# hku-mars/LiDAR_IMU_Init

Hardware: AMD Instinct MI355X
Metric: ICP+ESKF scans/sec @100k pts/scan (higher is better)
Workload: dtype f64; 1 GPU; stream100k: 100000 pts/scan (time-sorted) vs 1000000-pt local map, max_iteration 5, LIO mode (12-col H), static map, voxel-grid leaf 0.05; scans resident in HBM, 8 distinct scans cycled, the state reset to the scan's propagated state every step; map_points=1000000, params=harness/launch/ouster (reference-format yaml + launch), parallelism=points sharded x1, transport=none, rccl_ranks=0

## Files before the change

lidar_imu_init_amd/csrc/lii_capi.cpp:

```cpp
#include "lii_context.h"

using namespace lii_impl;

namespace lii_impl {

thread_local std::string g_err;

static constexpr unsigned kProfEventFlags = hipEventDisableSystemFence;

void harvest_knn_events(lii_handle h) {
  const unsigned int due = h->prof.ev_it_due;
  h->prof.ev_it_due = 0u;
  for (int it = 0; it < 16; it++) {
    if (!((due >> it) & 1u)) continue;
    float kk = 0;
    if (hipEventElapsedTime(&kk, h->prof.ev_it[2 * it], h->prof.ev_it[2 * it + 1]) != hipSuccess) continue;
    h->prof.timings[7] += kk;
    h->prof.timings[5] += 1;
  }
}

int fail(lii_handle h, int code, const std::string& msg) {
  if (h) h->err = msg;
  g_err = msg;
// ... 49 lines not shown
  return rb;
}
PoseArg pose_of(const lii_state& s) {
  PoseArg p;
  std::memcpy(p.R, s.rot_end, 72);
  std::memcpy(p.p, s.pos_end, 24);
  std::memcpy(p.RLI, s.offset_R_L_I, 72);
  std::memcpy(p.TLI, s.offset_T_L_I, 24);
  return p;
}
bool fuse_filter(lii_handle h, float leaf) {
  if (!(leaf > 0.f) || h->voxel_sort || h->no_fuse) return false;
  if (h->vh.part_world > 1) return true;
  return h->vh_mode == 1 && (h->vh_pinned || leaf == h->vh_leaf);
}
DeskewPlan deskew_plan(lii_handle h, const float4* in, float4* out, int n, bool sorted, const unsigned long long* extent, float leaf, bool fused,
                       DeskewCtrl ctrl) {
  DeskewPlan dp = {};
  dp.in = in; dp.out = out; dp.n = n; dp.sorted = sorted ? 1 : 0; dp.extent = extent; dp.bbox_rows = h->d_bbox_rows;
  dp.leaf = leaf; dp.vh = fused ? &h->vh : nullptr;
  if (ctrl == DeskewCtrl::pulled) { dp.ctrl_src = h->h_ctrl; dp.ctrl_dst = h->d_ctrl; dp.ctrl_bytes = (sizeof(IekfCtrl) + 15) / 16 * 16; }
#ifdef LII_GAP_TRACE
  if (ctrl != DeskewCtrl::none) dp.gap = h->d_gran;
#endif
  return dp;
}
int resolve_n_body(lii_handle h) {
  if (!h->n_body_pending) return LII_OK;
  int* v = h->h_small->n_body;
  HIPCHK(h, hipMemcpyAsync(v, h->d_nbody, 2 * sizeof(int), hipMemcpyDeviceToHost, h->stream));
  HIPCHK(h, hipStreamSynchronize(h->stream));
  h->n_body = v[0];
// ... 767 lines not shown
  unsigned int* mm = h->d_mm + 8 * h->mm_sel;
  if (h->bbox_rows == 0) {
    h->mm_sel ^= 1;
    launch_voxel_minmax(h->d_scan, n, mm, h->d_mm + 8 * h->mm_sel, s);
  }
  h->vh_calls++;
  if (h->vh_flag_pending && h->vh_calls >= h->vh_due) {
    HIPCHK(h, hipEventSynchronize(h->ev_vh));
    h->vh_flag_pending = false;
    if (h->vh_mode == 0 && *h->h_vh_crowded <= 32u) h->vh_mode = 1;
    else if (h->vh_mode == 1 && *h->h_vh_crowded > 64u) h->vh_mode = 0;
  }
  int hash_stages = 3;
  const bool inserted = h->vh_inserted;
  h->vh_inserted = false;
  if (inserted && leaf != h->vh_inserted_leaf) return fail(h, LII_ERR_STATE, "lii_downsample: the de-skew prepared the voxel filter for another leaf size");
  if (inserted) hash_stages = 4;
  if (!inserted && !h->vh_pinned && !h->voxel_sort && leaf != h->vh_leaf) {
    h->vh_leaf = leaf;
    h->vh_flag_pending = false;
    HIPCHK(h, hipMemsetAsync(h->vh.crowded, 0, sizeof(unsigned int), s));
    launch_voxel_hash(h->vh, h->d_scan, n, mm, h->d_bbox_rows, h->bbox_rows, leaf, h->d_body, h->d_nbody, h->d_nbody + 1, h->d_vpcl_out, 1, 0u, s);
    HIPCHK(h, hipMemcpyAsync(h->h_vh_crowded, h->vh.crowded, sizeof(unsigned int), hipMemcpyDeviceToHost, s));
    HIPCHK(h, hipMemsetAsync(h->vh.crowded, 0, sizeof(unsigned int), s));
    HIPCHK(h, hipStreamSynchronize(s));
    h->vh_mode = *h->h_vh_crowded > 32u ? 0 : 1;
    hash_stages = 2;
    if (h->vh_mode == 0)
      launch_voxel_hash_clear(h->vh, voxel_hash_slots(n), s);
  }
  const bool use_hash = inserted || (h->vh_mode == 1 && !h->voxel_sort);
  h->voxel_path_hash = use_hash;
  const bool by_voxel = inserted && h->vh.part_world > 1;
  if (use_hash) {
    if (++h->vh_epoch == 0u) h->vh_epoch = 1u;
    launch_voxel_hash(h->vh, h->d_scan, n, mm, h->d_bbox_rows, h->bbox_rows, leaf, h->d_body, h->d_nbody, h->d_nbody + 1, h->d_vpcl_out, hash_stages, h->vh_epoch, s, h->test_emit_late ? 1 : 0, inten, inten_out);
    if (!h->vh_pinned && !by_voxel && !h->vh_flag_pending && (++h->vh_watch & 15) == 0) {
      HIPCHK(h, hipMemcpyAsync(h->h_vh_crowded, h->vh.crowded, sizeof(unsigned int), hipMemcpyDeviceToHost, s));
      HIPCHK(h, hipMemsetAsync(h->vh.crowded, 0, sizeof(unsigned int), s));
      HIPCHK(h, hipEventRecord(h->ev_vh, s));
      h->vh_flag_pending = true;
      h->vh_due = h->vh_calls + 8;
    }
  } else {
    const VoxelSortPlan plan = voxel_sort_plan(n);
    launch_voxel_keys(h->d_scan, n, mm, h->d_bbox_rows, h->bbox_rows, leaf, h->d_vkeys_a, h->d_vpcl_in,
                      h->d_nbody + 1, plan.samples ? h->d_vsplit + 2048 : nullptr, plan.width, s);
    VoxelSortBuffers vb;
    vb.pcl_in = h->d_vpcl_in; vb.pcl_out = h->d_vpcl_out;
    vb.samples = h->d_vsplit + 2048;
    vb.keys_in = h->d_vkeys_a; vb.keys_out = h->d_vkeys_b; vb.idx_out = h->d_vidx_b;
// ... 150 lines not shown
```

lidar_imu_init_amd/csrc/lii_capi_register.cpp:

```cpp
#include "lii_context.h"
#include <cstddef>

#include "lii_hostmath.h"

using namespace lii_impl;

namespace {

int next_knn_epoch(lii_handle h) {
  h->knn_epoch = h->knn_epoch >= 0x3FFFFFFE ? 1 : h->knn_epoch + 1;
  return h->knn_epoch;
}
void launch_knn(lii_handle h, const GridView& g, const RegistrationBuffers& rb, const PoseArg* pose, int forced, int epoch,
                hipEvent_t ev_start = nullptr, hipEvent_t ev_stop = nullptr) {
  lii::launch_knn(g, rb, pose, h->d_ctrl, forced, h->d_ctrl->search_pose, h->stream, epoch, ev_start, ev_stop);
}

void note_noise_pass(lii_handle h) { if (h->noise.model == 1) h->noise.have_pass = true; }

int iterate(lii_handle h, const lii_state* st, bool search, bool imu_en, double* out91) {
  if (h->n_body <= 0) return fail(h, LII_ERR_STATE, "no down-sampled scan (call lii_downsample / lii_downsample_skip)");
  int rc = commit_map(h);
  if (rc != LII_OK) return rc;
  if (!search && !h->have_search) return fail(h, LII_ERR_STATE, "non-search iteration before any search");
// ... 102 lines not shown
void run_wait_hook(lii_handle h, bool inside) {
  if (!h->wait_hook) return;
  void (*hook)(void*) = h->wait_hook;
  h->wait_hook = nullptr;
  if (inside) h->in_wait_hook = true;
  hook(h->wait_hook_arg);
  if (inside) h->in_wait_hook = false;
}

struct DevicePasses {
  lii_handle h; const lii_iekf_opts* opts; hipStream_t s;
  GridView g; RegistrationBuffers rb;
  const PoseArg* pose;
  bool prof;
  unsigned int plan;

  int enqueue(int it) {
    const bool knn = it >= 16 || ((plan >> it) & 1u);
    const int epoch = knn ? next_knn_epoch(h) : 0;
    if (knn) {
      if (h->prof.kp_active) { const int r = kp_mark(h, LII_KP_KNN, it); if (r != LII_OK) return r; }
      if (prof && it < 16) launch_knn(h, g, rb, pose, -1, epoch, h->prof.ev_it[2 * it], h->prof.ev_it[2 * it + 1]);
      else launch_knn(h, g, rb, pose, -1, epoch);
    }
    if (h->prof.kp_active) { const int r = kp_mark(h, LII_KP_FIT, it); if (r != LII_OK) return r; }
    if (knn && h->wide_listed && !h->net.comm && h->net.n_ranks <= 1) launch_complete_listed(g, rb, h->d_ctrl, -1, s, epoch);
    launch_fit_reduce(g, rb, pose, h->d_ctrl, -1, opts->imu_en ? 1 : 0, h->cfg.plane_threshold, h->cfg.laser_point_cov_inv, s, epoch);
    note_noise_pass(h);
    if (h->prof.kp_active) { const int r = kp_mark(h, LII_KP_SOLVE, it); if (r != LII_OK) return r; }
    if (!h->net.comm) {
      launch_reduce_solve(rb, h->d_gran, h->d_ctrl, h->h_res, mailbox_view(h), s, epoch);
      return LII_OK;
    }
    launch_reduce91(rb, h->d_out91, h->d_ctrl, -1, s, epoch);
    ncclResult_t r = ncclAllReduce(h->d_out91, h->d_out91 + 128, kNormalEq, ncclDouble, ncclSum, h->net.comm, s);
    if (r != ncclSuccess) return fail(h, LII_ERR_COMM, std::string("ncclAllReduce: ") + ncclGetErrorString(r));
    launch_iekf_solve(h->d_ctrl, h->d_out91 + 128, h->h_res, s);
    return LII_OK;
  }

  int wait() {
    const int parked_word = h->update_seq | kLoopParked;
    if (h->poll_result && !h->net.comm) {
      volatile int* done = &h->h_res->done;
      unsigned int spins = 0;
// ... 136 lines not shown
  if (!h->ctrl_preloaded) {
    if (h->staging_busy) HIPCHK(h, hipStreamSynchronize(s));
    fill_ctrl(h, state, state_prop, opts);
    HIPCHK(h, hipMemcpyAsync(h->d_ctrl, h->h_ctrl, sizeof(IekfCtrl), hipMemcpyHostToDevice, s));
  }
  h->ctrl_preloaded = false;
  h->h_res->singular = 0; h->h_res->it = -1;
  if (h->lm.in_job) {
    rc = local_map_enqueue(h, h->d_ctrl->st + 9, nullptr, h->prof.kp_active);
    if (rc != LII_OK) return rc;
  }
  const bool prof = h->prof.profiling && h->prof.prof_mode != 3;
  DevicePasses p = {h, opts, s, grid_view(h), reg_buffers(h), reinterpret_cast<const PoseArg*>(h->d_ctrl), prof, h->plan_cur};
  if (prof) harvest_knn_events(h);
  const unsigned int plan0 = p.plan;
  const auto t_loop0 = std::chrono::steady_clock::now();
  for (int it = 0; it < opts->max_iterations; it++) {
    if (it < 16 && !((p.plan >> (16 + it)) & 1u)) break;
    rc = p.enqueue(it);
    if (rc != LII_OK) return rc;
  }
  if (h->diag) h->prof.host_loop_enq_us = std::chrono::duration<double, std::micro>(std::chrono::steady_clock::now() - t_loop0).count();
  if (h->prof.kp_active) { rc = kp_mark(h, LII_KP_KINDS); if (rc != LII_OK) return rc; }
  h->map_enqueued_early = false;
  if (h->map_after_update && !h->net.comm && !h->prof.profiling) {
    const auto t_me0 = std::chrono::steady_clock::now();
    h->map_enqueued_early = map_update_early(h) == 1;
    p.g = grid_view(h);
    if (h->diag) h->prof.host_map_us[1] += std::chrono::duration<double, std::micro>(std::chrono::steady_clock::now() - t_me0).count();
  }
  if (h->pub.any()) { rc = publish_enqueue(h, h->d_ctrl, nullptr, true); if (rc != LII_OK) return rc; }
  prearm_arm(h);
  run_wait_hook(h, true);
  bool parked_once = false;
  rc = p.wait();
  if (rc == LII_OK) rc = p.continue_parked(&parked_once);
  if (rc != LII_OK) return rc;
  if (h->pub.any() && parked_once) {
// ... 255 lines not shown
    src_dev = nullptr;
  }
  const float4* const src4 = static_cast<const float4*>(src_dev);
  if (feed || cv) {
    rc = feed ? imu_prologue(h, jv, &job->opts, feed, state, adopt, src4, n_next) : cv_prologue(h, jv, &job->opts, cv, state, adopt, src4, n_next);
    if (rc != LII_OK) { h->prof.kp_active = false; return rc; }
  } else {
    const int rc_now = fast ? fast_prologue(h, jv, &job->opts, state, state_prop, adopt, src4, n_next, use_pre, &rc)
                            : general_prologue(h, jv, &job->opts, state, state_prop, adopt, src_dev, src_n, n_next, &rc);
    if (rc_now != LII_OK) return rc_now;
  }
  if (h->ctrl_preloaded && h->ctrl_pending) {
    HIPCHK(h, hipMemcpyAsync(h->d_ctrl, h->h_ctrl, h->ctrl_pending, hipMemcpyHostToDevice, h->stream));
    h->ctrl_pending = 0;
  }
  if (rc == LII_OK) rc = jv.leaf > 0 ? lii_downsample(h, jv.leaf, nullptr, nullptr) : lii_downsample_skip(h, nullptr);
  const auto t_pre = std::chrono::steady_clock::now();
  h->map_after_update = jv.map_update && !h->host_solve;
  h->map_enqueued_early = false;
  h->wait_hook = rc == LII_OK ? jv.while_waiting : nullptr;
  h->wait_hook_arg = jv.while_waiting_arg;
  h->lm.in_job = local_map && rc == LII_OK;
  if (rc == LII_OK) rc = lii_iekf_update(h, state, state_prop ? state_prop : state, &job->opts, report);
  if (h->lm.in_job) {
    if (rc == LII_OK) local_map_settle(h);
    else h->lm.counts_pending = true;
    h->lm.in_job = false;
  }
  run_wait_hook(h, false);
  h->map_after_update = false;
  if (rc == LII_OK && jv.map_update && !h->map_enqueued_early) rc = lii_map_incremental(h, state, nullptr, nullptr);
  h->map_enqueued_early = false;
  h->poses_preloaded = h->ctrl_preloaded = false;
  h->prof.kp_active = false;
  note_host_times(h, t_entry, t_first, t_pre);
  lii_state* const prop_out = feed ? feed->prop_out : (cv ? cv->prop_out : nullptr);
  if (rc == LII_OK && prop_out) std::memcpy(prop_out, h->imu.h_out.get(), sizeof(lii_state));
  return rc;
// ... 200 lines not shown
```

lidar_imu_init_amd/csrc/lii_context.h:

```cpp
#pragma once
#include <hip/hip_runtime_api.h>
#include <rccl/rccl.h>

#include <algorithm>
#include <atomic>
#include <chrono>
#include <cmath>
#include <cstdio>
#include <cstdlib>
#include <cstring>
#include <string>
#include <vector>

#include "../../include/liinit_hip.h"
#include "lii_launch.h"
#include "lii_owned.h"

using lii::BlockEntry; using lii::IekfCtrl; using lii::IekfResult; using lii::PoseArg; using lii::VoxelHashBuffers; using lii::MailboxHost;
using lii::DevBuf; using lii::PinnedBuf;
constexpr size_t kCtrlBytes = (sizeof(lii::IekfCtrl) + 255) / 256 * 256;

constexpr int kMapBoxesMax = 4096;
constexpr int kImuSamplesMax = 63;
constexpr int kGxRanksMax = 128;
// ... 167 lines not shown
  size_t ctrl_pending = 0;
  bool extent_valid = false;
  DevBuf<unsigned int> d_bbox_rows;
  int bbox_rows = 0;
  DevBuf<unsigned long long> d_vkeys_a, d_vkeys_b;
  DevBuf<unsigned int> d_vidx_b;
  DevBuf<unsigned long long> d_vcomp, d_vsplit;
  DevBuf<unsigned int> d_vhist;
  DevBuf<unsigned short> d_vbucket;
  DevBuf<unsigned int> d_vpcl_in, d_vpcl_out;
  VoxelHashBuffers vh = {};
  DevBuf<unsigned char> vh_slots;
  DevBuf<unsigned int> vh_slot_of, vh_next, vh_crowded;
  DevBuf<unsigned long long> vh_counts;
  unsigned int vh_epoch = 0;
  bool voxel_sort = false;
  bool vh_pinned = false;
  float fuse_leaf = 0.f;
  float vh_inserted_leaf = 0.f;
  bool vh_inserted = false;
  int vh_mode = 1;
  float vh_leaf = -1.f;
  unsigned int vh_watch = 0;
  unsigned long long vh_calls = 0, vh_due = 0;
  bool voxel_path_hash = false;
  PinnedBuf<unsigned int> h_vh_crowded;
  lii::Event ev_vh;
  bool vh_flag_pending = false;
  bool body_partitioned = false;
  bool body_reordered = false;
// ... 184 lines not shown
using namespace lii;

int fail(lii_handle h, int code, const std::string& msg);
inline unsigned int next_pow2(unsigned int v) {
  unsigned int p = 1;
  while (p < v) p <<= 1;
  return p;
}
int kp_mark(lii_handle h, int kind, int it = 0);
void harvest_knn_events(lii_handle h);
GridView grid_view(const lii_context* c);
RegistrationBuffers reg_buffers(const lii_context* c);
PoseArg pose_of(const lii_state& s);
int resolve_n_body(lii_handle h);
bool fuse_filter(lii_handle h, float leaf);
enum class DeskewCtrl { none, ahead, pulled };
DeskewPlan deskew_plan(lii_handle h, const float4* in, float4* out, int n, bool sorted, const unsigned long long* extent, float leaf, bool fused,
                       DeskewCtrl ctrl);
int pcl_order(lii_handle h, const int** perm);
void extent_discard(lii_handle h);
int scan_sort_into(lii_handle h, const float4* src, int n);
void intensity_detach(lii_handle h);
int intensity_buffers(lii_handle h);
int scan_materialize(lii_handle h);
bool gate_move(lii::GateState* st, unsigned long long seq, unsigned long long to);
void prearm_cancel(lii_handle h);
void prearm_arm(lii_handle h);
bool prearm_go(lii_handle h, const lii_state* state, const lii_pose6d* poses, int K);
unsigned long long* extent_of_scan(lii_handle h);
MailboxView mailbox_view(lii_handle h);
// ... 37 lines not shown
```

lidar_imu_init_amd/csrc/lii_device.h:

```cpp
#pragma once
#include <hip/hip_runtime.h>
#include <stdint.h>

namespace lii {

constexpr int kMatch = 5;
constexpr int kNeedy = 0x100;
constexpr int kDone = 0x400;
constexpr int kCountMask = 0xFF;
constexpr int kCovered = 0x200;
constexpr int kBlock = 256;
constexpr int kNormalEq = 91;
constexpr int kCoarseShift = 3;
constexpr unsigned long long kEmptyKey = ~0ull;
constexpr int kCellBias = 1 << 20;
constexpr int kVoxIdxBits = 28;
constexpr int kVoxKeyBits = 36;
constexpr unsigned long long kVoxDropKey = (1ull << kVoxKeyBits) - 1ull;

constexpr int kMapCtrUsed = 0, kMapCtrValid = 1, kMapCtrBlocks = 2, kMapCtrWork = 3, kMapCtrOverflow = 4, kMapCtrEvents = 5, kMapCtrDropped = 6, kMapCtrSlots = 7, kMapCtrWinStale = 8 , kMapCtrTicket = 15 , kMapCtrWords = 16;

__device__ __forceinline__ void mat3_mul(const double A[9], const double B[9], double C[9]) {
#pragma unroll
  for (int r = 0; r < 3; r++)
// ... 357 lines not shown
constexpr int kLoopParked = 0x40000000;
struct IekfResult {
  double st[kStateDoubles];
  double ne[96];
  int it, searches, effect_num, converged, singular;
  int done;
  int parked_it;
  int part_overflow;
  int search_log[16];
  int parked_search;
  int unfinished;
  long long ts[16];
  long long ts0[16];
};

}
```

lidar_imu_init_amd/csrc/lii_iekf.hip:

```cpp
#include <hip/hip_runtime.h>
#include <string.h>
#include <cstring>
#include <math.h>

#include "lii_device.h"
#include "lii_launch.h"

namespace lii {

constexpr int N = 24;
constexpr int H = 12;
constexpr int LDH = 13;

__device__ __forceinline__ double readlane_f64(double v, int lane) {
  union { double d; int i[2]; } u;
  u.d = v;
  u.i[0] = __builtin_amdgcn_readlane(u.i[0], lane);
  u.i[1] = __builtin_amdgcn_readlane(u.i[1], lane);
  return u.d;
}
__device__ __forceinline__ bool gj12_pivoting(double (&col)[H]) {
#pragma unroll
  for (int k = 0; k < H; k++) {
    double mx = 0.0;
// ... 395 lines not shown

__device__ __attribute__((noinline, used)) void solve_code_end();
__device__ __forceinline__ int warm_code() {
  const char* pc = reinterpret_cast<const char*>(__builtin_amdgcn_s_getpc() & ~63ull);
  const char* end = reinterpret_cast<const char*>(&solve_code_end);
  int acc = 0;
  if (threadIdx.x < 192) {
#pragma unroll
    for (int u = 0; u < 3; u++) {
      const char* a = pc + (size_t)(threadIdx.x + 192 * u) * 64;
      if (a + 64 <= end) acc ^= *reinterpret_cast<const volatile int*>(a);
    }
  }
  return acc;
}
__device__ __forceinline__ unsigned int pass_tag(int seq, int it) { return ((unsigned int)seq << 6) ^ (unsigned int)(it + 1); }
__global__ __launch_bounds__(kSolveThreads) void k_reduce_solve(const double* __restrict__ partials, int n_blocks, int stride,
                                                                 unsigned long long* __restrict__ gran, IekfCtrl* c, IekfResult* res,
                                                                 MailboxView mb, const int* __restrict__ flag_count) {
  __shared__ double s_w[kSolveThreads / 64];
  const int stop = c->stop, seq = c->seq, it = c->it;
  const int t = blockIdx.x;
  if (t < kNormalEq) {
    const double acc = final_sum_row<kSolveThreads>(partials + (size_t)t * stride, n_blocks, s_w);
    if (stop) return;
    if (threadIdx.x == 0 && !(mb.test_drop_sum && t == 5)) {
      const unsigned int tag = pass_tag(seq, it);
      const unsigned long long b = (unsigned long long)__double_as_longlong(acc);
      __hip_atomic_store(gran + 2 * t, ((unsigned long long)tag << 32) | (b & 0xFFFFFFFFull), __ATOMIC_RELAXED, __HIP_MEMORY_SCOPE_AGENT);
      __hip_atomic_store(gran + 2 * t + 1, ((unsigned long long)tag << 32) | (b >> 32), __ATOMIC_RELAXED, __HIP_MEMORY_SCOPE_AGENT);
    }
    return;
  }
  if (stop) return;
  if (threadIdx.x == kSolveThreads - 1 && flag_count) {
    const int now = max(flag_count[0], flag_count[1]);
    const int before = it == 0 ? 0 : (int)gran[240];
    const int um = max(now, before);
    gran[240] = (unsigned long long)um;
    res_store(&res->unfinished, um);
  }
  const unsigned int tag = pass_tag(seq, it);
  const int warm = warm_code();
  iekf_solve_body(c, res, [&](double* s_ne) {
    __shared__ int s_mb_ok;
    if (threadIdx.x < 64) {
// ... 43 lines not shown

__device__ __attribute__((noinline, used)) void solve_code_end() { asm volatile("s_nop 0"); }

__global__ __launch_bounds__(64) void k_mailbox_allreduce(double* out, MailboxView mb) {
  const int l = threadIdx.x;
  double v0 = l < kNormalEq ? out[l] : 0.0, v1 = l + 64 < kNormalEq ? out[l + 64] : 0.0;
  const bool ok = mailbox_allreduce(mb, v0, v1);
  if (l < kNormalEq) out[l] = ok ? v0 : __builtin_nan("");
  if (l + 64 < kNormalEq) out[l + 64] = ok ? v1 : __builtin_nan("");
}

void launch_mailbox_allreduce(double* out91, const MailboxView& mb, hipStream_t s) {
  hipLaunchKernelGGL(k_mailbox_allreduce, dim3(1), dim3(64), 0, s, out91, mb);
}
void launch_reduce_solve(const RegistrationBuffers& rb, unsigned long long* gran, IekfCtrl* c, IekfResult* res, const MailboxView& mb,
                         hipStream_t s, int epoch) {
  const int bound = rb.shard_world > 1 ? (rb.n + rb.shard_world - 1) / rb.shard_world + 1 : rb.n;
  int nb = (bound + kBlock - 1) / kBlock;
  if (nb < 1) nb = 1;
  nb += completion_blocks(epoch);
  hipLaunchKernelGGL(k_reduce_solve, dim3(kNormalEq + 1), dim3(kSolveThreads), 0, s, rb.partials, nb, rb.partial_stride, gran, c, res, mb, rb.flag_count);
}
__global__ void k_loop_resume(IekfCtrl* c, unsigned int plan_mask) {
  c->stop = 0;
  c->plan_mask = plan_mask;
}
void launch_loop_resume(IekfCtrl* c, unsigned int plan_mask, hipStream_t s) { hipLaunchKernelGGL(k_loop_resume, dim3(1), dim3(1), 0, s, c, plan_mask); }
void launch_iekf_solve(IekfCtrl* c, const double* ne, IekfResult* res, hipStream_t s) {
  hipLaunchKernelGGL(k_iekf_solve, dim3(1), dim3(kSolveThreads), 0, s, c, ne, res);
}

}
```

lidar_imu_init_amd/csrc/lii_launch.h:

```cpp
#pragma once
#include <hip/hip_runtime_api.h>
#include <stddef.h>

#include <string>

#include "lii_device.h"
#include "lii_fov.h"

struct lii_context;
int lii_internal_fail(lii_context* h, int code, const std::string& msg);
#define HIPCHK(h, call)                                                                                            \
  do {                                                                                                             \
    hipError_t e_ = (call);                                                                                        \
    if (e_ != hipSuccess) return lii_internal_fail(h, LII_ERR_HIP, std::string(#call) + ": " + hipGetErrorString(e_)); \
  } while (0)
int lii_internal_scan_defer(lii_context* h, const void* dev_float4, int32_t n);
int lii_internal_scan_materialize(lii_context* h);
int lii_internal_in_wait_hook(lii_context* h);
int lii_internal_scan_is_deferred(lii_context* h);
int lii_internal_intensity_refused(lii_context* h);
int lii_internal_scan_intensity_adopt(lii_context* h, const float* dev_float, int32_t n);
void lii_internal_prearm_cancel(lii_context* h);
hipStream_t lii_internal_stream(lii_context* h);
void** lii_internal_ingest_slot(lii_context* h);
// ... 28 lines not shown
size_t sort_u64_bits_temp_bytes(size_t n, int end_bit);
void sort_pairs_u64_bits(void* temp, size_t temp_bytes, const unsigned long long* kin, unsigned long long* kout, const unsigned int* vin,
                         unsigned int* vout, size_t n, int end_bit, hipStream_t s);
void launch_knn(const GridView& g, const RegistrationBuffers& rb, const PoseArg* pose,
                const IekfCtrl* ctrl, int forced, double* search_pose_out, hipStream_t s, int epoch,
                hipEvent_t ev_start = nullptr, hipEvent_t ev_stop = nullptr);
#ifdef LII_FALLBACK_TRACE
void fb_trace_read(unsigned long long out[32]);
#endif
void launch_knn_complete(const GridView& g, const RegistrationBuffers& rb, hipStream_t s);
void launch_complete_listed(const GridView& g, const RegistrationBuffers& rb, const IekfCtrl* ctrl, int forced, hipStream_t s, int epoch);
void launch_fit_reduce(const GridView& g, const RegistrationBuffers& rb, const PoseArg* pose,
                       const IekfCtrl* ctrl, int forced, int imu_en, double plane_thr, double rinv, hipStream_t s, int epoch);
void launch_reduce91(const RegistrationBuffers& rb, double* out91, const IekfCtrl* ctrl, int forced, hipStream_t s, int epoch);
void launch_reduce_solve(const RegistrationBuffers& rb, unsigned long long* gran, IekfCtrl* c, IekfResult* res, const MailboxView& mb,
                         hipStream_t s, int epoch);
void launch_mailbox_allreduce(double* out91, const MailboxView& mb, hipStream_t s);
struct MailboxHost {
  void* map = nullptr;
  size_t bytes = 0;
  double* dev_slots = nullptr;
  bool registered = false;
  char name[64] = {0};
  double* own = nullptr;
  double* peer_ptr[64] = {nullptr};
  double** d_peers = nullptr;
  int n_peers = 0;
  unsigned char** d_gather_peers = nullptr;
  size_t gather_block = 0;
  int gather_cap = 0;
};
// ... 18 lines not shown
void launch_voxel_minmax(const float4* pts, int n, unsigned int* mm, unsigned int* mm_next, hipStream_t s);
void launch_voxel_keys(const float4* pts, int n, const unsigned int* mm, const unsigned int* bbox_rows, int n_rows, float leaf,
                       unsigned long long* keys, unsigned int* pcl_keys, int* filtered_dev,
                       unsigned long long* samples, int sample_width, hipStream_t s);
struct VoxelHashBuffers {
  void* slots;
  unsigned int *slot_of, *next;
  unsigned long long* counts;
  unsigned int* crowded;
  int part_world, part_rank;
  int* part_overflow;
};
size_t voxel_hash_slots(int max_n);
int voxel_partition_bound(int n, int world);
void launch_voxel_hash_clear(const VoxelHashBuffers& vh, size_t slots, hipStream_t s);
void launch_voxel_hash(const VoxelHashBuffers& vh, const float4* pts, int n, const unsigned int* mm, const unsigned int* bbox_rows,
                       int n_rows, float leaf, float4* out, int* n_out, int* filtered, unsigned int* pcl_out, int stages, unsigned int epoch,
                       hipStream_t s, int test_late = 0 ,
                       const float* inten = nullptr, float* inten_out = nullptr);
struct DeskewPlan {
  const float4* in;
  float4* out;
  int n;
  int sorted;
  const unsigned long long* extent;
  unsigned int* bbox_rows;
  float leaf;
  const VoxelHashBuffers* vh;
  const void* ctrl_src;
  void* ctrl_dst;
// ... 188 lines not shown
```

lidar_imu_init_amd/csrc/lii_scan.hip:

```cpp
#include <hip/hip_runtime.h>
#include <string.h>
#include <cstring>
#include <math.h>
#include <stdint.h>

#include "lii_device.h"
#include "lii_imu_dev.h"
#include "lii_launch.h"

namespace lii {

#ifdef LII_FRONT_TRACE
__device__ unsigned long long g_front_trace[32];
__device__ __forceinline__ long long* ft_lds() {
  __shared__ long long s_ft[8];
  return s_ft;
}
#define LII_FT(k) do { if (threadIdx.x == 0) ft_lds()[k] = wall_clock64(); } while (0)
#define LII_FT_W(k) do { if (threadIdx.x == 0) { asm volatile("s_waitcnt vmcnt(0)" ::: "memory"); ft_lds()[k] = wall_clock64(); } } while (0)
__device__ __forceinline__ void ft_flush(int base) {
  if (threadIdx.x != 0) return;
  const long long* s = ft_lds();
  atomicAdd(&g_front_trace[base], 1ull);
  long long last = s[0];
// ... 680 lines not shown
    unsigned int hsh = j * 2654435761u;
    hsh ^= hsh >> 15; hsh *= 2246822519u; hsh ^= hsh >> 13;
    const unsigned int w = min((unsigned int)sample_width, (unsigned int)n - lo);
    if (lo + hsh % w == (unsigned int)i) samples[j] = (key << kVoxIdxBits) | (unsigned long long)(unsigned int)i;
  }
}
__global__ __launch_bounds__(256) void k_vh_clear(VhSlot* slots, unsigned int n_slots) {
  const unsigned int i = blockIdx.x * blockDim.x + threadIdx.x;
  if (i >= n_slots) return;
  VhSlot s;
  s.key = ~0ull; s.first = kVhEmpty; s.creator = kVhEmpty; s.count = 0u; s.head = kVhEmpty; s.pad = 0u;
#pragma unroll
  for (int k = 0; k < kVhMembers - 1; k++) s.members[k] = kVhEmpty;
  slots[i] = s;
}
__device__ __forceinline__ void fold_bbox_rows(const unsigned int* __restrict__ bbox_rows, int n_rows, unsigned int* s_mm ) {
  unsigned int lo[3] = {0xFFFFFFFFu, 0xFFFFFFFFu, 0xFFFFFFFFu}, hi[3] = {0, 0, 0};
  for (int r = threadIdx.x; r < n_rows; r += 256) {
    const uint4 a = *reinterpret_cast<const uint4*>(bbox_rows + r * 8), b = *reinterpret_cast<const uint4*>(bbox_rows + r * 8 + 4);
    lo[0] = min(lo[0], a.x); lo[1] = min(lo[1], a.y); lo[2] = min(lo[2], a.z);
    hi[0] = max(hi[0], b.x); hi[1] = max(hi[1], b.y); hi[2] = max(hi[2], b.z);
  }
  block_bbox_reduce(lo, hi);
  if (threadIdx.x < 3) { s_mm[threadIdx.x] = lo[0]; s_mm[3 + threadIdx.x] = hi[0]; }
  __syncthreads();
}
struct BoxRows { uint4 a0, b0, a1, b1; };
__device__ __forceinline__ uint4 box_row_half(const unsigned int* p ) {
  const unsigned long long* q = reinterpret_cast<const unsigned long long*>(p);
  const unsigned long long u = __hip_atomic_load(q, __ATOMIC_RELAXED, __HIP_MEMORY_SCOPE_WAVEFRONT), w = __hip_atomic_load(q + 1, __ATOMIC_RELAXED, __HIP_MEMORY_SCOPE_WAVEFRONT);
// ... 100 lines not shown
  unsigned int total;
  const unsigned int rank = block_rank_of_flag(first, s_w, &total);
  const bool hold = test_late != 0 && (blockIdx.x % 7u) == 3u && !(ABS && v.identity && !ident_part);
  if (tid == 0 && !hold) __hip_atomic_store(counts + blockIdx.x, ((unsigned long long)epoch << 32) | total, __ATOMIC_RELAXED, __HIP_MEMORY_SCOPE_AGENT);
  LII_FT(4);
  if (ABS && !fold_first) {
    fold_bbox_rows_finish(box_rows, bbox_rows, n_rows, s_mm);
    v = voxel_prepare(s_mm, leaf);
    if (i == 0) *filtered = v.identity ? 0 : 1;
    LII_FT(3);
  }
  if (ABS && v.identity && !ident_part) {
    if (in_range) { out[i] = p0; pcl_out[i] = (unsigned)i; }
    if (INT && in_range) inten_out[i] = q0;
    if (blockIdx.x == gridDim.x - 1 && tid == 0) *n_out = n;
    if (first) {
      uint4* line = reinterpret_cast<uint4*>(sl);
      line[0] = make_uint4(0xFFFFFFFFu, 0xFFFFFFFFu, kVhEmpty, kVhEmpty);
      line[1] = make_uint4(0u, kVhEmpty, kVhEmpty, kVhEmpty);
    }
    return;
  }
  float4 cen = make_float4(0.f, 0.f, 0.f, 0.f);
  float cen_i = 0.f;
  if (first) {
    const unsigned int cnt = ident_part ? 1u : hd.y + 1u;
    float sx = __fadd_rn(0.f, p0.x), sy = __fadd_rn(0.f, p0.y), sz = __fadd_rn(0.f, p0.z), st = __fadd_rn(0.f, p0.w);
    float si = INT ? __fadd_rn(0.f, q0) : 0.f;
    unsigned int m[kVhMembers] = {m0.x, m0.y, m0.z, m0.w, m1.x, m1.y, m1.z, m1.w, m2.x, m2.y};
#pragma unroll
    for (int k = 0; k < kVhMembers; k++)
      if ((unsigned)k >= cnt) m[k] = kVhEmpty;
    if (cnt > 512u) {
#pragma unroll
      for (int k = 0; k < kVhMembers; k++) {
// ... 30 lines not shown
      prefix_below(counts, epoch, (int)blockIdx.x, s_sum, test_late != 0, [&](int q) -> unsigned int {
    const int j = q * 256 + tid;
    bool f = false;
    if (j < n) {
      const unsigned int sq = tb.slot_of[j];
      if (sq != kVhEmpty) {
        const uint4 a = *reinterpret_cast<const uint4*>(tb.slots + sq);
        f = ident_part || min(a.z, a.w) == (unsigned)j;
      }
    }
    unsigned int tot;
    (void)block_rank_of_flag(f, s_w, &tot);
    return tot;
  }).y;
  LII_FT(6);
  if (hold) {
    if (tid == 0) {
      __hip_atomic_store(counts + blockIdx.x, ((unsigned long long)epoch << 32) | total, __ATOMIC_RELAXED, __HIP_MEMORY_SCOPE_AGENT);
      __builtin_amdgcn_fence(__ATOMIC_RELEASE, "agent");
    }
    __syncthreads();
  }
  if (blockIdx.x == gridDim.x - 1 && tid == 0) {
    int n_down = (int)(base + total);
    if (ABS && tb.part_world > 1u && n_down > tb.part_bound) {
      n_down = tb.part_bound;
      __hip_atomic_store(tb.part_overflow, 1, __ATOMIC_RELAXED, __HIP_MEMORY_SCOPE_SYSTEM);
    }
    *n_out = n_down;
  }
  if (first) {
    const unsigned int pos = base + rank;
    out[pos] = cen;
    if (INT) inten_out[pos] = cen_i;
    if (ident_part) {
      pcl_out[pos] = (unsigned)i;
    } else if (ABS) {
      const int i0 = (int)(floorf(p0.x * v.inv_leaf) - (float)v.min_b[0]);
      const int i1 = (int)(floorf(p0.y * v.inv_leaf) - (float)v.min_b[1]);
      const int i2 = (int)(floorf(p0.z * v.inv_leaf) - (float)v.min_b[2]);
      pcl_out[pos] = (unsigned)(i0 * v.mul[0] + i1 * v.mul[1] + i2 * v.mul[2]);
    } else {
      pcl_out[pos] = (unsigned int)key;
    }
    uint4* line = reinterpret_cast<uint4*>(sl);
    line[0] = make_uint4(0xFFFFFFFFu, 0xFFFFFFFFu, kVhEmpty, kVhEmpty);
    line[1] = make_uint4(0u, kVhEmpty, kVhEmpty, kVhEmpty);
  }
  LII_FT_W(7);
  LII_FT_END(16);
}

static inline int nblk(int n, int b) { return (n + b - 1) / b; }
void launch_time_extent(const float4* pts, int n, unsigned long long* extent, unsigned long long* extent_next, float4* copy_to,
                        const void* ctrl_src, void* ctrl_dst, size_t ctrl_bytes, hipStream_t s) {
  int nb = nblk(n, 256 * 2);
  if (nb > 256) nb = 256;
  if (nb < 1) nb = 1;
  hipLaunchKernelGGL(k_time_extent, dim3(nb + (ctrl_bytes ? 1 : 0)), dim3(256), 0, s, pts, n, extent, extent_next, copy_to,
                     static_cast<const uint4*>(ctrl_src), static_cast<uint4*>(ctrl_dst), (int)(ctrl_bytes / 16));
}
void launch_sort_keys(const float4* pts, int n, unsigned int* key, unsigned int* idx, hipStream_t s) {
// ... 100 lines not shown
  else hipLaunchKernelGGL(k_deskew_cv<false>, dim3(nb), dim3(256), 0, s, io, a);
}
void launch_deskew_cv_prop(const DeskewPlan& p, const CvFuseH& fh, hipStream_t s) {
  if (p.n <= 0) return;
  CvFuseArg f;
  static_assert(sizeof(CvFuseArg) == sizeof(CvFuseH), "layout");
  memcpy(&f, &fh, sizeof(f));
  const DeskewIo io = deskew_io(p);
  const int nb = nblk(p.n, 256) + 1;
  if (p.vh) hipLaunchKernelGGL(k_deskew_cv_prop<true>, dim3(nb), dim3(256), 0, s, io, f);
  else hipLaunchKernelGGL(k_deskew_cv_prop<false>, dim3(nb), dim3(256), 0, s, io, f);
}
void launch_voxel_hash_clear(const VoxelHashBuffers& vh, size_t slots, hipStream_t s) {
  hipLaunchKernelGGL(k_vh_clear, dim3((unsigned int)((slots + 255) / 256)), dim3(256), 0, s, static_cast<VhSlot*>(vh.slots), (unsigned int)slots);
}
void launch_voxel_hash(const VoxelHashBuffers& vh, const float4* pts, int n, const unsigned int* mm, const unsigned int* bbox_rows,
                       int n_rows, float leaf, float4* out, int* n_out, int* filtered, unsigned int* pcl_out, int stages, unsigned int epoch,
                       hipStream_t s, int test_late, const float* inten, float* inten_out) {
  if (n <= 0) return;
  const bool wi = inten != nullptr && inten_out != nullptr;
  const VhTable tb = vh_table(&vh, n, (stages & 4) != 0);
  const int nb = nblk(n, 256);
  if (stages & 1) hipLaunchKernelGGL(k_vhash_insert, dim3(nb), dim3(256), 0, s, pts, n, mm, bbox_rows, n_rows, leaf, tb, filtered);
  const float* const no_in = nullptr;
  float* const no_out = nullptr;
  if ((stages & 2) && !wi) hipLaunchKernelGGL((k_vhash_emit<false, false>), dim3(nb), dim3(256), 0, s, pts, n, tb, vh.counts, epoch, out, n_out, pcl_out, nullptr, 0, leaf, filtered, test_late, no_in, no_out);
  if ((stages & 2) && wi) hipLaunchKernelGGL((k_vhash_emit<false, true>), dim3(nb), dim3(256), 0, s, pts, n, tb, vh.counts, epoch, out, n_out, pcl_out, nullptr, 0, leaf, filtered, test_late, inten, inten_out);
  if ((stages & 4) && !wi) hipLaunchKernelGGL((k_vhash_emit<true, false>), dim3(nb), dim3(256), 0, s, pts, n, tb, vh.counts, epoch, out, n_out, pcl_out, bbox_rows, n_rows, leaf, filtered, test_late, no_in, no_out);
  if ((stages & 4) && wi) hipLaunchKernelGGL((k_vhash_emit<true, true>), dim3(nb), dim3(256), 0, s, pts, n, tb, vh.counts, epoch, out, n_out, pcl_out, bbox_rows, n_rows, leaf, filtered, test_late, inten, inten_out);
}
// ... 14 lines not shown
```

Before: 7921 scans/s.

## Defer voxel-hash slot release into extra blocks of the reduce-solve kernel

Removes the per-slot hash-table reset stores from the voxel-hash emit kernel and tracks how many points still owe a release. The release is done later by extra rider blocks appended to the last planned reduce-solve launch, or by a standalone release kernel when no such launch is available. This drops a fence and a __syncthreads from the emit kernel's critical path and hides the slot clearing behind the small solve kernel. In exchange it adds bookkeeping that must settle the release before the next hash use, and it relies on the slot field offsets fixed by a static_assert.

Measured after the change: 7967 scans/s (median of 6 runs). Within noise of the previous version (+0.6%).

```diff
diff --git a/lidar_imu_init_amd/csrc/lii_capi.cpp b/lidar_imu_init_amd/csrc/lii_capi.cpp
--- a/lidar_imu_init_amd/csrc/lii_capi.cpp
+++ b/lidar_imu_init_amd/csrc/lii_capi.cpp
@@ -87,8 +87,18 @@
   if (h->vh.part_world > 1) return true;
   return h->vh_mode == 1 && (h->vh_pinned || leaf == h->vh_leaf);
 }
+lii::VhRelease vh_release_take(lii_handle h) {
+  const lii::VhRelease r = {h->vh.slot_of, h->vh_owed_n, h->vh.slots};
+  h->vh_owed_n = 0;
+  return r;
+}
+void vh_release_settle(lii_handle h) {
+  if (h->vh_owed_n <= 0) return;
+  launch_voxel_hash_release(vh_release_take(h), h->stream);
+}
 DeskewPlan deskew_plan(lii_handle h, const float4* in, float4* out, int n, bool sorted, const unsigned long long* extent, float leaf, bool fused,
                        DeskewCtrl ctrl) {
+  if (fused) vh_release_settle(h);
   DeskewPlan dp = {};
   dp.in = in; dp.out = out; dp.n = n; dp.sorted = sorted ? 1 : 0; dp.extent = extent; dp.bbox_rows = h->d_bbox_rows;
   dp.leaf = leaf; dp.vh = fused ? &h->vh : nullptr;
@@ -886,8 +896,10 @@
   int hash_stages = 3;
   const bool inserted = h->vh_inserted;
   h->vh_inserted = false;
+  if (inserted && leaf != h->vh_inserted_leaf) { h->vh_owed_n = n; vh_release_settle(h); }
   if (inserted && leaf != h->vh_inserted_leaf) return fail(h, LII_ERR_STATE, "lii_downsample: the de-skew prepared the voxel filter for another leaf size");
   if (inserted) hash_stages = 4;
+  if (!inserted) vh_release_settle(h);
   if (!inserted && !h->vh_pinned && !h->voxel_sort && leaf != h->vh_leaf) {
     h->vh_leaf = leaf;
     h->vh_flag_pending = false;
@@ -907,6 +919,8 @@
   if (use_hash) {
     if (++h->vh_epoch == 0u) h->vh_epoch = 1u;
     launch_voxel_hash(h->vh, h->d_scan, n, mm, h->d_bbox_rows, h->bbox_rows, leaf, h->d_body, h->d_nbody, h->d_nbody + 1, h->d_vpcl_out, hash_stages, h->vh_epoch, s, h->test_emit_late ? 1 : 0, inten, inten_out);
+    h->vh_owed_n = n;
+    if (!h->vh_release_deferred) vh_release_settle(h);
     if (!h->vh_pinned && !by_voxel && !h->vh_flag_pending && (++h->vh_watch & 15) == 0) {
       HIPCHK(h, hipMemcpyAsync(h->h_vh_crowded, h->vh.crowded, sizeof(unsigned int), hipMemcpyDeviceToHost, s));
       HIPCHK(h, hipMemsetAsync(h->vh.crowded, 0, sizeof(unsigned int), s));
diff --git a/lidar_imu_init_amd/csrc/lii_capi_register.cpp b/lidar_imu_init_amd/csrc/lii_capi_register.cpp
--- a/lidar_imu_init_amd/csrc/lii_capi_register.cpp
+++ b/lidar_imu_init_amd/csrc/lii_capi_register.cpp
@@ -140,6 +140,7 @@
   const PoseArg* pose;
   bool prof;
   unsigned int plan;
+  int release_it = -1;
 
   int enqueue(int it) {
     const bool knn = it >= 16 || ((plan >> it) & 1u);
@@ -155,6 +156,10 @@
     note_noise_pass(h);
     if (h->prof.kp_active) { const int r = kp_mark(h, LII_KP_SOLVE, it); if (r != LII_OK) return r; }
     if (!h->net.comm) {
+      if (it == release_it && h->vh_owed_n > 0) {
+        launch_reduce_solve(rb, h->d_gran, h->d_ctrl, h->h_res, mailbox_view(h), s, epoch, vh_release_take(h));
+        return LII_OK;
+      }
       launch_reduce_solve(rb, h->d_gran, h->d_ctrl, h->h_res, mailbox_view(h), s, epoch);
       return LII_OK;
     }
@@ -321,6 +326,10 @@
   DevicePasses p = {h, opts, s, grid_view(h), reg_buffers(h), reinterpret_cast<const PoseArg*>(h->d_ctrl), prof, h->plan_cur};
   if (prof) harvest_knn_events(h);
   const unsigned int plan0 = p.plan;
+  for (int it = 0; it < opts->max_iterations; it++) {
+    if (it < 16 && !((p.plan >> (16 + it)) & 1u)) break;
+    p.release_it = it;
+  }
   const auto t_loop0 = std::chrono::steady_clock::now();
   for (int it = 0; it < opts->max_iterations; it++) {
     if (it < 16 && !((p.plan >> (16 + it)) & 1u)) break;
@@ -329,6 +338,7 @@
   }
   if (h->diag) h->prof.host_loop_enq_us = std::chrono::duration<double, std::micro>(std::chrono::steady_clock::now() - t_loop0).count();
   if (h->prof.kp_active) { rc = kp_mark(h, LII_KP_KINDS); if (rc != LII_OK) return rc; }
+  vh_release_settle(h);
   h->map_enqueued_early = false;
   if (h->map_after_update && !h->net.comm && !h->prof.profiling) {
     const auto t_me0 = std::chrono::steady_clock::now();
@@ -614,7 +624,9 @@
     HIPCHK(h, hipMemcpyAsync(h->d_ctrl, h->h_ctrl, h->ctrl_pending, hipMemcpyHostToDevice, h->stream));
     h->ctrl_pending = 0;
   }
+  h->vh_release_deferred = true;
   if (rc == LII_OK) rc = jv.leaf > 0 ? lii_downsample(h, jv.leaf, nullptr, nullptr) : lii_downsample_skip(h, nullptr);
+  h->vh_release_deferred = false;
   const auto t_pre = std::chrono::steady_clock::now();
   h->map_after_update = jv.map_update && !h->host_solve;
   h->map_enqueued_early = false;
@@ -622,6 +634,7 @@
   h->wait_hook_arg = jv.while_waiting_arg;
   h->lm.in_job = local_map && rc == LII_OK;
   if (rc == LII_OK) rc = lii_iekf_update(h, state, state_prop ? state_prop : state, &job->opts, report);
+  vh_release_settle(h);
   if (h->lm.in_job) {
     if (rc == LII_OK) local_map_settle(h);
     else h->lm.counts_pending = true;
diff --git a/lidar_imu_init_amd/csrc/lii_context.h b/lidar_imu_init_amd/csrc/lii_context.h
--- a/lidar_imu_init_amd/csrc/lii_context.h
+++ b/lidar_imu_init_amd/csrc/lii_context.h
@@ -205,6 +205,8 @@
   DevBuf<unsigned int> vh_slot_of, vh_next, vh_crowded;
   DevBuf<unsigned long long> vh_counts;
   unsigned int vh_epoch = 0;
+  int vh_owed_n = 0;
+  bool vh_release_deferred = false;
   bool voxel_sort = false;
   bool vh_pinned = false;
   float fuse_leaf = 0.f;
@@ -419,6 +421,8 @@
 PoseArg pose_of(const lii_state& s);
 int resolve_n_body(lii_handle h);
 bool fuse_filter(lii_handle h, float leaf);
+void vh_release_settle(lii_handle h);
+lii::VhRelease vh_release_take(lii_handle h);
 enum class DeskewCtrl { none, ahead, pulled };
 DeskewPlan deskew_plan(lii_handle h, const float4* in, float4* out, int n, bool sorted, const unsigned long long* extent, float leaf, bool fused,
                        DeskewCtrl ctrl);
diff --git a/lidar_imu_init_amd/csrc/lii_device.h b/lidar_imu_init_amd/csrc/lii_device.h
--- a/lidar_imu_init_amd/csrc/lii_device.h
+++ b/lidar_imu_init_amd/csrc/lii_device.h
@@ -395,4 +395,17 @@
   long long ts0[16];
 };
 
-}
+struct VhRelease {
+  const unsigned int* slot_of;
+  int n;
+  void* slots;
+};
+__device__ __forceinline__ void vh_release_point(const VhRelease& r, int i) {
+  const unsigned int slot = r.slot_of[i];
+  if (slot == 0xFFFFFFFFu) return;
+  uint4* line = static_cast<uint4*>(r.slots) + 4 * (size_t)slot;
+  line[0] = make_uint4(0xFFFFFFFFu, 0xFFFFFFFFu, 0xFFFFFFFFu, 0xFFFFFFFFu);
+  line[1] = make_uint4(0u, 0xFFFFFFFFu, 0xFFFFFFFFu, 0xFFFFFFFFu);
+}
+
+}
diff --git a/lidar_imu_init_amd/csrc/lii_iekf.hip b/lidar_imu_init_amd/csrc/lii_iekf.hip
--- a/lidar_imu_init_amd/csrc/lii_iekf.hip
+++ b/lidar_imu_init_amd/csrc/lii_iekf.hip
@@ -433,10 +433,11 @@
   }
   return acc;
 }
+constexpr int kReleaseRiders = 160;
 __device__ __forceinline__ unsigned int pass_tag(int seq, int it) { return ((unsigned int)seq << 6) ^ (unsigned int)(it + 1); }
 __global__ __launch_bounds__(kSolveThreads) void k_reduce_solve(const double* __restrict__ partials, int n_blocks, int stride,
                                                                  unsigned long long* __restrict__ gran, IekfCtrl* c, IekfResult* res,
-                                                                 MailboxView mb, const int* __restrict__ flag_count) {
+                                                                 MailboxView mb, const int* __restrict__ flag_count, VhRelease release) {
   __shared__ double s_w[kSolveThreads / 64];
   const int stop = c->stop, seq = c->seq, it = c->it;
   const int t = blockIdx.x;
@@ -449,6 +450,11 @@
       __hip_atomic_store(gran + 2 * t, ((unsigned long long)tag << 32) | (b & 0xFFFFFFFFull), __ATOMIC_RELAXED, __HIP_MEMORY_SCOPE_AGENT);
       __hip_atomic_store(gran + 2 * t + 1, ((unsigned long long)tag << 32) | (b >> 32), __ATOMIC_RELAXED, __HIP_MEMORY_SCOPE_AGENT);
     }
+    return;
+  }
+  if (t > kNormalEq) {
+    const int riders = (int)gridDim.x - (kNormalEq + 1);
+    for (int i = (t - (kNormalEq + 1)) * kSolveThreads + (int)threadIdx.x; i < release.n; i += riders * kSolveThreads) vh_release_point(release, i);
     return;
   }
   if (stop) return;
@@ -522,12 +528,15 @@
   hipLaunchKernelGGL(k_mailbox_allreduce, dim3(1), dim3(64), 0, s, out91, mb);
 }
 void launch_reduce_solve(const RegistrationBuffers& rb, unsigned long long* gran, IekfCtrl* c, IekfResult* res, const MailboxView& mb,
-                         hipStream_t s, int epoch) {
+                         hipStream_t s, int epoch, const VhRelease& release) {
   const int bound = rb.shard_world > 1 ? (rb.n + rb.shard_world - 1) / rb.shard_world + 1 : rb.n;
   int nb = (bound + kBlock - 1) / kBlock;
   if (nb < 1) nb = 1;
   nb += completion_blocks(epoch);
-  hipLaunchKernelGGL(k_reduce_solve, dim3(kNormalEq + 1), dim3(kSolveThreads), 0, s, rb.partials, nb, rb.partial_stride, gran, c, res, mb, rb.flag_count);
+  int riders = release.n > 0 ? (release.n + kSolveThreads - 1) / kSolveThreads : 0;
+  if (riders > kReleaseRiders) riders = kReleaseRiders;
+  hipLaunchKernelGGL(k_reduce_solve, dim3(kNormalEq + 1 + riders), dim3(kSolveThreads), 0, s, rb.partials, nb, rb.partial_stride, gran, c, res, mb, rb.flag_count,
+                     release);
 }
 __global__ void k_loop_resume(IekfCtrl* c, unsigned int plan_mask) {
   c->stop = 0;
diff --git a/lidar_imu_init_amd/csrc/lii_launch.h b/lidar_imu_init_amd/csrc/lii_launch.h
--- a/lidar_imu_init_amd/csrc/lii_launch.h
+++ b/lidar_imu_init_amd/csrc/lii_launch.h
@@ -66,7 +66,7 @@
                        const IekfCtrl* ctrl, int forced, int imu_en, double plane_thr, double rinv, hipStream_t s, int epoch);
 void launch_reduce91(const RegistrationBuffers& rb, double* out91, const IekfCtrl* ctrl, int forced, hipStream_t s, int epoch);
 void launch_reduce_solve(const RegistrationBuffers& rb, unsigned long long* gran, IekfCtrl* c, IekfResult* res, const MailboxView& mb,
-                         hipStream_t s, int epoch);
+                         hipStream_t s, int epoch, const VhRelease& release = VhRelease{nullptr, 0, nullptr});
 void launch_mailbox_allreduce(double* out91, const MailboxView& mb, hipStream_t s);
 struct MailboxHost {
   void* map = nullptr;
@@ -115,6 +115,7 @@
 size_t voxel_hash_slots(int max_n);
 int voxel_partition_bound(int n, int world);
 void launch_voxel_hash_clear(const VoxelHashBuffers& vh, size_t slots, hipStream_t s);
+void launch_voxel_hash_release(const VhRelease& r, hipStream_t s);
 void launch_voxel_hash(const VoxelHashBuffers& vh, const float4* pts, int n, const unsigned int* mm, const unsigned int* bbox_rows,
                        int n_rows, float leaf, float4* out, int* n_out, int* filtered, unsigned int* pcl_out, int stages, unsigned int epoch,
                        hipStream_t s, int test_late = 0 ,
diff --git a/lidar_imu_init_amd/csrc/lii_scan.hip b/lidar_imu_init_amd/csrc/lii_scan.hip
--- a/lidar_imu_init_amd/csrc/lii_scan.hip
+++ b/lidar_imu_init_amd/csrc/lii_scan.hip
@@ -718,6 +718,12 @@
   for (int k = 0; k < kVhMembers - 1; k++) s.members[k] = kVhEmpty;
   slots[i] = s;
 }
+static_assert(offsetof(VhSlot, key) == 0 && offsetof(VhSlot, first) == 8 && offsetof(VhSlot, creator) == 12 && offsetof(VhSlot, count) == 16 &&
+              offsetof(VhSlot, head) == 20 && offsetof(VhSlot, members) == 24, "vh_release_point writes the first 32 bytes of a slot by position");
+__global__ __launch_bounds__(256) void k_vh_release(VhRelease r) {
+  const int i = blockIdx.x * blockDim.x + threadIdx.x;
+  if (i < r.n) vh_release_point(r, i);
+}
 __device__ __forceinline__ void fold_bbox_rows(const unsigned int* __restrict__ bbox_rows, int n_rows, unsigned int* s_mm ) {
   unsigned int lo[3] = {0xFFFFFFFFu, 0xFFFFFFFFu, 0xFFFFFFFFu}, hi[3] = {0, 0, 0};
   for (int r = threadIdx.x; r < n_rows; r += 256) {
@@ -848,11 +854,6 @@
     if (in_range) { out[i] = p0; pcl_out[i] = (unsigned)i; }
     if (INT && in_range) inten_out[i] = q0;
     if (blockIdx.x == gridDim.x - 1 && tid == 0) *n_out = n;
-    if (first) {
-      uint4* line = reinterpret_cast<uint4*>(sl);
-      line[0] = make_uint4(0xFFFFFFFFu, 0xFFFFFFFFu, kVhEmpty, kVhEmpty);
-      line[1] = make_uint4(0u, kVhEmpty, kVhEmpty, kVhEmpty);
-    }
     return;
   }
   float4 cen = make_float4(0.f, 0.f, 0.f, 0.f);
@@ -913,13 +914,7 @@
     return tot;
   }).y;
   LII_FT(6);
-  if (hold) {
-    if (tid == 0) {
-      __hip_atomic_store(counts + blockIdx.x, ((unsigned long long)epoch << 32) | total, __ATOMIC_RELAXED, __HIP_MEMORY_SCOPE_AGENT);
-      __builtin_amdgcn_fence(__ATOMIC_RELEASE, "agent");
-    }
-    __syncthreads();
-  }
+  if (hold && tid == 0) __hip_atomic_store(counts + blockIdx.x, ((unsigned long long)epoch << 32) | total, __ATOMIC_RELAXED, __HIP_MEMORY_SCOPE_AGENT);
   if (blockIdx.x == gridDim.x - 1 && tid == 0) {
     int n_down = (int)(base + total);
     if (ABS && tb.part_world > 1u && n_down > tb.part_bound) {
@@ -942,9 +937,6 @@
     } else {
       pcl_out[pos] = (unsigned int)key;
     }
-    uint4* line = reinterpret_cast<uint4*>(sl);
-    line[0] = make_uint4(0xFFFFFFFFu, 0xFFFFFFFFu, kVhEmpty, kVhEmpty);
-    line[1] = make_uint4(0u, kVhEmpty, kVhEmpty, kVhEmpty);
   }
   LII_FT_W(7);
   LII_FT_END(16);
@@ -1075,6 +1067,9 @@
 void launch_voxel_hash_clear(const VoxelHashBuffers& vh, size_t slots, hipStream_t s) {
   hipLaunchKernelGGL(k_vh_clear, dim3((unsigned int)((slots + 255) / 256)), dim3(256), 0, s, static_cast<VhSlot*>(vh.slots), (unsigned int)slots);
 }
+void launch_voxel_hash_release(const VhRelease& r, hipStream_t s) {
+  if (r.n > 0) hipLaunchKernelGGL(k_vh_release, dim3(nblk(r.n, 256)), dim3(256), 0, s, r);
+}
 void launch_voxel_hash(const VoxelHashBuffers& vh, const float4* pts, int n, const unsigned int* mm, const unsigned int* bbox_rows,
                        int n_rows, float leaf, float4* out, int* n_out, int* filtered, unsigned int* pcl_out, int stages, unsigned int epoch,
                        hipStream_t s, int test_late, const float* inten, float* inten_out) {
```
